# henrycharlesworth/settlers_of_catan_RL

Measured on AMD Instinct MI355X. Metric: Catan env-steps/sec at 65k parallel games, higher is better.
Workload: dtype u8/u32 (integer bitboards); 1 GPU; configs[1]: 65 536 parallel envs per GPU, random policy, step+mask only, bit-exact vs CPU oracle; games_per_gpu=65536, games_total=65536, validate_actions=True, auto_reset=True, parallelism=games sharded over 1 GPU(s), no collective

## Files before the change

settlers_of_catan_rl_amd/csrc/catan_kernels.hip:

```cpp
#include <hip/hip_runtime.h>
#include <stdint.h>

#include "catan_state.h"

#define CATAN_TABLE static __device__ __constant__ const
#define CATAN_FN static __device__ __forceinline__
#define CATAN_TOPOLOGY_CODE
#include "catan_topology.inc"

namespace catan {

#define DEVI __device__ __forceinline__

constexpr int BLOCK = 256;
constexpr u64 ALL54 = (1ull << 54) - 1;

constexpr int MT_RING = 8192, MT_AHEAD = 6144, MT_AHEAD_PY = 1024;
struct MtGen { u32 mt[624]; u32 idx; u32 produced; u32 ring[MT_RING]; };
struct MtPair { MtGen np, py; u32 cons_py; };
struct BoardCfg {
    int32_t randomise;
    int32_t fixed_terrain;
    int32_t fixed_numbers;
    int8_t terrain[19];
    int8_t numbers[18];
    int8_t pad_[7];
};
constexpr int MAX_BOARD_CFGS = 16;
struct Ctx {
    u32* R;
    long N;
    long n;
    u32 key0, key1;
    u64 env_id0;
    MtPair* mt;
    const BoardCfg* bcfg;
    const u8* bcfg_idx;
};

template <class D>
struct StOps {
// ... 1053 lines not shown
    const long i = (long)blockIdx.x * BLOCK + threadIdx.x;
    if (i >= rows * MASK_BITS) return;
    const long r = i / MASK_BITS;
    const int j = (int)(i - r * MASK_BITS);
    const long e = games != nullptr ? (long)games[r] : r;
    float v;
    if (e < 0 || e >= n || (busy != nullptr && busy[e] != 0)) v = j == M0 + T_ENDTURN ? 1.0f : 0.0f;
    else v = (float)((mpk[e * MPK_STRIDE + (j >> 5)] >> (j & 31)) & 1u);
    out[i] = v;
}

__global__ __launch_bounds__(BLOCK) void k_copy_masks11(const u32* __restrict__ mpk, long n, u32* __restrict__ out) {
    const long i = (long)blockIdx.x * BLOCK + threadIdx.x;
    if (i >= n * 11) return;
    const long e = i / 11;
    out[i] = mpk[e * MPK_STRIDE + (int)(i - e * 11)];
}
__global__ __launch_bounds__(256) void k_masked_row_store(unsigned char* __restrict__ dst, const unsigned char* __restrict__ src,
                                                          const long long* __restrict__ t, const unsigned char* __restrict__ sel,
                                                          long row_bytes, long step_stride_bytes) {
    const long r = blockIdx.x;
    if (!sel[r]) return;
    unsigned char* d = dst + t[r] * step_stride_bytes + r * row_bytes;
    const unsigned char* s = src + r * row_bytes;
    if ((((unsigned long long)d | (unsigned long long)s | (unsigned long long)row_bytes) & 3) == 0) {
        for (long i = threadIdx.x; i < row_bytes / 4; i += 256) reinterpret_cast<u32*>(d)[i] = reinterpret_cast<const u32*>(s)[i];
    } else if ((((unsigned long long)d | (unsigned long long)s | (unsigned long long)row_bytes) & 1) == 0) {
        for (long i = threadIdx.x; i < row_bytes / 2; i += 256) reinterpret_cast<unsigned short*>(d)[i] = reinterpret_cast<const unsigned short*>(s)[i];
    } else {
        for (long i = threadIdx.x; i < row_bytes; i += 256) d[i] = s[i];
    }
}

DEVI int nth_set(u64 v, int nth) {
    if (nth >= __popcll(v)) return -1;
    int pos = 0;
    u32 w = (u32)v;
    int c = __popc(w);
    if (nth >= c) { nth -= c; w = (u32)(v >> 32); pos = 32; }
    c = __popc(w & 0xFFFFu); if (nth >= c) { nth -= c; w >>= 16; pos += 16; }
    c = __popc(w & 0xFFu);   if (nth >= c) { nth -= c; w >>= 8;  pos += 8; }
    c = __popc(w & 0xFu);    if (nth >= c) { nth -= c; w >>= 4;  pos += 4; }
    c = __popc(w & 0x3u);    if (nth >= c) { nth -= c; w >>= 2;  pos += 2; }
    if (nth >= (int)(w & 1u)) pos += 1;
    return pos;
}
DEVI int pick64(u64 v, u32 w) {
    int k = __popcll(v);
    if (k == 0) return 0;
    return nth_set(v, (int)__umulhi(w, (u32)k));
}
template <class S>
DEVI int sample_random(const Ctx& c, const S& s, const u32 (&m)[MASK_WORDS], u32 step_idx, int (&a)[ACTION_WORDS],
                       u32* __restrict__ pctr, u8* __restrict__ busy, int tag_now, int tag_now2) {
#pragma unroll
    for (int i = 0; i < ACTION_WORDS; i++) a[i] = 0;
    if (pctr != nullptr) {
        const u32 own = pctr[s.e];
        int b = busy[s.e];
        if (b >= 2 && (b == tag_now || b == tag_now2)) { busy[s.e] = 0; b = 0; }
        if (b) { a[0] = -1; return -1; }
        step_idx = own;
        pctr[s.e] = step_idx + 1;
    }
    u64 id = c.env_id0 + (u64)s.e;
    u32 w[8];
    {
        u32 o[4];
        philox4x32_10(2 * step_idx, 1u, (u32)id, (u32)(id >> 32), c.key0, c.key1, o);
        w[0] = o[0]; w[1] = o[1]; w[2] = o[2]; w[3] = o[3];
    }
    int t = pick64(getr<M0, 13>(m), w[0]);
    a[0] = t;
    switch (t) {
    case T_SETTLE: a[1] = pick64(getr<M1, 54>(m), w[1]); break;
    case T_CITY: a[1] = pick64(getr<M1 + 54, 54>(m), w[1]); break;
    case T_ROAD: {
        u64 lo = getr<M2, 64>(m), hi = getr<M2 + 64, 9>(m);
        int k = __popcll(lo) + __popcll(hi);
        int nth = k ? (int)__umulhi(w[1], (u32)k) : 0;
        int nlo = __popcll(lo);
        a[2] = k == 0 ? 0 : (nth < nlo ? nth_set(lo, nth) : 64 + nth_set(hi, nth - nlo));
        break;
    }
    case T_ROBBER: a[3] = pick64(getr<M3, 19>(m), w[1]); break;
    case T_PLAYDEV:
        a[4] = pick64(getr<M4, 5>(m), w[1]);
        if (a[4] == C_MONO) a[15] = pick64(getr<M9 + 10, 5>(m), w[2]);
        else if (a[4] == C_YOP) { a[15] = pick64(getr<M9 + 15, 5>(m), w[2]); a[16] = pick64(getr<M10, 5>(m), w[3]); }
        break;
    case T_EXCHANGE: a[15] = pick64(getr<M9, 5>(m), w[1]); a[16] = pick64(getr<M10, 5>(m), w[2]); break;
    case T_PROPOSE: {
        {
            u32 o[4];
            philox4x32_10(2 * step_idx + 1, 1u, (u32)id, (u32)(id >> 32), c.key0, c.key1, o);
            w[4] = o[0]; w[5] = o[1]; w[6] = o[2]; w[7] = o[3];
        }
        int pid = s.b(B_GO);
        int hand[5], tot = 0;
#pragma unroll
        for (int r = 0; r < 5; r++) { hand[r] = s.res(pid, r); tot += hand[r]; }
        a[6] = (int)__umulhi(w[1], 3u);
        int n_give = 1 + (int)(w[2] & 1u), n_recv = 1 + (int)((w[2] >> 1) & 1u);
        if (n_give > tot) n_give = tot;
#pragma unroll
        for (int i = 0; i < 2; i++) if (i < n_give) {
            int nth = (int)__umulhi(w[3 + i], (u32)tot), r = 0;
            bool found = false;
#pragma unroll
            for (int k = 0; k < 5; k++) if (!found) { if (nth < hand[k]) { r = k; found = true; } else nth -= hand[k]; }
            a[7 + i] = r + 1;
#pragma unroll
            for (int k = 0; k < 5; k++) hand[k] -= (k == r) ? 1 : 0;
            tot--;
        }
#pragma unroll
        for (int i = 0; i < 2; i++) if (i < n_recv) a[11 + i] = 1 + (int)__umulhi(w[5 + i], 5u);
        break;
    }
    case T_RESPOND: a[5] = pick64(getr<M5, 2>(m), w[1]); break;
    case T_STEAL: a[6] = pick64(getr<M6 + 3, 3>(m), w[1]); break;
    case T_DISCARD: a[17] = pick64(getr<M11, 5>(m), w[1]); break;
    default: break;
    }
    return t;
}
template <class S>
DEVI bool action_valid(const S& s, const int (&a)[ACTION_WORDS]) {
    const int t = a[0];
    if (t < 0 || t > 12) return false;
    int cnt[5] = { 0, 0, 0, 0, 0 };
    if (t == T_STEAL && (a[6] < 0 || a[6] > 2)) return false;
    if (t == T_PLAYDEV) {
        if (a[4] == C_MONO && (a[15] < 0 || a[15] > 4)) return false;
        if (a[4] == C_YOP && (a[15] < 0 || a[15] > 4 || a[16] < 0 || a[16] > 4)) return false;
    }
    if (t == T_EXCHANGE && (a[15] < 0 || a[15] > 4 || a[16] < 0 || a[16] > 4)) return false;
    if (t == T_PROPOSE) {
        if (a[6] < 0 || a[6] > 2) return false;
        bool stop = false;
#pragma unroll
        for (int i = 0; i < 4; i++) {
            const int v = a[7 + i];
            if (v == 0) stop = true;
            if (!stop) {
                if (v < 0 || v > 5) return false;
#pragma unroll
                for (int k = 0; k < 5; k++) cnt[k] += (k == v - 1) ? 1 : 0;
            }
        }
        stop = false;
#pragma unroll
        for (int i = 0; i < 4; i++) { const int v = a[11 + i]; if (v == 0) stop = true; if (!stop && (v < 0 || v > 5)) return false; }
    }
    if (t == T_RESPOND && (a[5] < 0 || a[5] > 1)) return false;
    if (t == T_DISCARD && (a[17] < 0 || a[17] > 4)) return false;
// ... 1756 lines not shown
```

settlers_of_catan_rl_amd/csrc/catan_topology.inc:

```
CATAN_TABLE uint8_t TILE_CORNER[19][6] = {
  {0, 1, 2, 3, 4, 5},
  {6, 5, 4, 7, 8, 9},
  {10, 9, 8, 11, 12, 13},
  {2, 14, 15, 16, 17, 3},
  {4, 3, 17, 18, 19, 7},
  {8, 7, 19, 20, 21, 11},
  {12, 11, 21, 22, 23, 24},
  {15, 25, 26, 27, 28, 16},
  {17, 16, 28, 29, 30, 18},
  {19, 18, 30, 31, 32, 20},
  {21, 20, 32, 33, 34, 22},
  {23, 22, 34, 35, 36, 37},
  {28, 27, 38, 39, 40, 29},
  {30, 29, 40, 41, 42, 31},
  {32, 31, 42, 43, 44, 33},
  {34, 33, 44, 45, 46, 35},
  {40, 39, 47, 48, 49, 41},
  {42, 41, 49, 50, 51, 43},
  {44, 43, 51, 52, 53, 45},
};
CATAN_TABLE uint8_t EDGE_CORNER[72][2] = {
  {2, 3},
  {3, 4},
  {1, 2},
// ... 214 lines not shown
  {9, 13, 14},
  {9, 10, 14},
  {10, 14, 15},
  {10, 11, 15},
  {11, 15, 255},
  {11, 255, 255},
  {11, 255, 255},
  {12, 255, 255},
  {12, 16, 255},
  {12, 13, 16},
  {13, 16, 17},
  {13, 14, 17},
  {14, 17, 18},
  {14, 15, 18},
  {15, 18, 255},
  {15, 255, 255},
  {16, 255, 255},
  {16, 255, 255},
  {16, 17, 255},
  {17, 255, 255},
  {17, 18, 255},
  {18, 255, 255},
  {18, 255, 255},
};
CATAN_TABLE uint8_t CORNER_HSLOT[54] = {0, 0, 255, 255, 255, 255, 1, 255, 255, 1, 255, 255, 2, 255, 8, 8, 255, 255, 255, 255, 255, 255, 255, 255, 2, 255, 255, 7, 255, 255, 255, 255, 255, 255, 255, 255, 3, 3, 7, 255, 255, 255, 255, 255, 255, 4, 4, 6, 6, 255, 5, 5, 255, 255};
CATAN_TABLE uint8_t PLACEMENT[19] = {0, 3, 7, 12, 16, 17, 18, 15, 11, 6, 2, 1, 4, 8, 13, 14, 10, 5, 9};
CATAN_TABLE uint32_t TILE_NBR_MASK[19] = {0x1au, 0x35u, 0x62u, 0x191u, 0x32bu, 0x656u, 0xc24u, 0x1108u, 0x3298u, 0x6530u, 0xca60u, 0x8440u, 0x12180u, 0x35300u, 0x6a600u, 0x44c00u, 0x23000u, 0x56000u, 0x2c000u};
CATAN_TABLE uint64_t TILE_CORNER_MASK[19] = {0x3full, 0x3f0ull, 0x3f00ull, 0x3c00cull, 0xe0098ull, 0x380980ull, 0x1e01800ull, 0x1e018000ull, 0x70070000ull, 0x1c01c0000ull, 0x700700000ull, 0x3c00c00000ull, 0x1c038000000ull, 0x700e0000000ull, 0x1c0380000000ull, 0x700e00000000ull, 0x3838000000000ull, 0xe0e0000000000ull, 0x38380000000000ull};
CATAN_TABLE uint64_t CORNER_NBR_MASK[54] = {0x22ull, 0x5ull, 0x400aull, 0x20014ull, 0xa8ull, 0x51ull, 0x220ull, 0x80110ull, 0xa80ull, 0x540ull, 0x2200ull, 0x201100ull, 0x1002800ull, 0x1400ull, 0x8004ull, 0x2014000ull, 0x10028000ull, 0x50008ull, 0x400a0000ull, 0x140080ull, 0x100280000ull, 0x500800ull, 0x400a00000ull, 0x2001400000ull, 0x801000ull, 0x4008000ull, 0xa000000ull, 0x4014000000ull, 0x28010000ull, 0x10050000000ull, 0xa0040000ull, 0x40140000000ull, 0x280100000ull, 0x100500000000ull, 0xa00400000ull, 0x401400000000ull, 0x2800000000ull, 0x1000800000ull, 0x8008000000ull, 0x814000000000ull, 0x28020000000ull, 0x2050000000000ull, 0xa0080000000ull, 0x8140000000000ull, 0x280200000000ull, 0x20500000000000ull, 0x200800000000ull, 0x1008000000000ull, 0x2800000000000ull, 0x5020000000000ull, 0xa000000000000ull, 0x14080000000000ull, 0x28000000000000ull, 0x10200000000000ull};
CATAN_TABLE uint64_t EDGE_CORNER_MASK[72] = {0xcull, 0x18ull, 0x6ull, 0x30ull, 0x3ull, 0x21ull, 0x90ull, 0x180ull, 0x300ull, 0x60ull, 0x240ull, 0x900ull, 0x1800ull, 0x3000ull, 0x600ull, 0x2400ull, 0x18000ull, 0x30000ull, 0xc000ull, 0x20008ull, 0x4004ull, 0x60000ull, 0xc0000ull, 0x80080ull, 0x180000ull, 0x300000ull, 0x200800ull, 0x600000ull, 0xc00000ull, 0x1800000ull, 0x1001000ull, 0xc000000ull, 0x18000000ull, 0x6000000ull, 0x10010000ull, 0x2008000ull, 0x30000000ull, 0x60000000ull, 0x40040000ull, 0xc0000000ull, 0x180000000ull, 0x100100000ull, 0x300000000ull, 0x600000000ull, 0x400400000ull, 0xc00000000ull, 0x1800000000ull, 0x3000000000ull, 0x2000800000ull, 0xc000000000ull, 0x18000000000ull, 0x4008000000ull, 0x10020000000ull, 0x30000000000ull, 0x60000000000ull, 0x40080000000ull, 0xc0000000000ull, 0x180000000000ull, 0x100200000000ull, 0x300000000000ull, 0x600000000000ull, 0x400800000000ull, 0x1800000000000ull, 0x3000000000000ull, 0x808000000000ull, 0x2020000000000ull, 0x6000000000000ull, 0xc000000000000ull, 0x8080000000000ull, 0x18000000000000ull, 0x30000000000000ull, 0x20200000000000ull};
#ifdef CATAN_TOPOLOGY_CODE
CATAN_FN uint64_t topo_blocked(uint64_t occ) {
    const uint32_t ol = (uint32_t)occ, oh = (uint32_t)(occ >> 32);
    uint32_t bl = ol, bh = oh, m;
    m = 0u - ((ol >> 0) & 1u); bl |= m & 0x22u;
    m = 0u - ((ol >> 1) & 1u); bl |= m & 0x5u;
    m = 0u - ((ol >> 2) & 1u); bl |= m & 0x400au;
    m = 0u - ((ol >> 3) & 1u); bl |= m & 0x20014u;
    m = 0u - ((ol >> 4) & 1u); bl |= m & 0xa8u;
    m = 0u - ((ol >> 5) & 1u); bl |= m & 0x51u;
    m = 0u - ((ol >> 6) & 1u); bl |= m & 0x220u;
    m = 0u - ((ol >> 7) & 1u); bl |= m & 0x80110u;
    m = 0u - ((ol >> 8) & 1u); bl |= m & 0xa80u;
    m = 0u - ((ol >> 9) & 1u); bl |= m & 0x540u;
    m = 0u - ((ol >> 10) & 1u); bl |= m & 0x2200u;
    m = 0u - ((ol >> 11) & 1u); bl |= m & 0x201100u;
    m = 0u - ((ol >> 12) & 1u); bl |= m & 0x1002800u;
    m = 0u - ((ol >> 13) & 1u); bl |= m & 0x1400u;
    m = 0u - ((ol >> 14) & 1u); bl |= m & 0x8004u;
    m = 0u - ((ol >> 15) & 1u); bl |= m & 0x2014000u;
    m = 0u - ((ol >> 16) & 1u); bl |= m & 0x10028000u;
    m = 0u - ((ol >> 17) & 1u); bl |= m & 0x50008u;
    m = 0u - ((ol >> 18) & 1u); bl |= m & 0x400a0000u;
    m = 0u - ((ol >> 19) & 1u); bl |= m & 0x140080u;
    m = 0u - ((ol >> 20) & 1u); bl |= m & 0x280000u; bh |= m & 0x1u;
    m = 0u - ((ol >> 21) & 1u); bl |= m & 0x500800u;
    m = 0u - ((ol >> 22) & 1u); bl |= m & 0xa00000u; bh |= m & 0x4u;
    m = 0u - ((ol >> 23) & 1u); bl |= m & 0x1400000u; bh |= m & 0x20u;
    m = 0u - ((ol >> 24) & 1u); bl |= m & 0x801000u;
    m = 0u - ((ol >> 25) & 1u); bl |= m & 0x4008000u;
    m = 0u - ((ol >> 26) & 1u); bl |= m & 0xa000000u;
    m = 0u - ((ol >> 27) & 1u); bl |= m & 0x14000000u; bh |= m & 0x40u;
    m = 0u - ((ol >> 28) & 1u); bl |= m & 0x28010000u;
    m = 0u - ((ol >> 29) & 1u); bl |= m & 0x50000000u; bh |= m & 0x100u;
    m = 0u - ((ol >> 30) & 1u); bl |= m & 0xa0040000u;
    m = 0u - ((ol >> 31) & 1u); bl |= m & 0x40000000u; bh |= m & 0x401u;
    m = 0u - ((oh >> 0) & 1u); bl |= m & 0x80100000u; bh |= m & 0x2u;
    m = 0u - ((oh >> 1) & 1u); bh |= m & 0x1005u;
    m = 0u - ((oh >> 2) & 1u); bl |= m & 0x400000u; bh |= m & 0xau;
    m = 0u - ((oh >> 3) & 1u); bh |= m & 0x4014u;
    m = 0u - ((oh >> 4) & 1u); bh |= m & 0x28u;
    m = 0u - ((oh >> 5) & 1u); bl |= m & 0x800000u; bh |= m & 0x10u;
    m = 0u - ((oh >> 6) & 1u); bl |= m & 0x8000000u; bh |= m & 0x80u;
    m = 0u - ((oh >> 7) & 1u); bh |= m & 0x8140u;
    m = 0u - ((oh >> 8) & 1u); bl |= m & 0x20000000u; bh |= m & 0x280u;
    m = 0u - ((oh >> 9) & 1u); bh |= m & 0x20500u;
    m = 0u - ((oh >> 10) & 1u); bl |= m & 0x80000000u; bh |= m & 0xa00u;
    m = 0u - ((oh >> 11) & 1u); bh |= m & 0x81400u;
    m = 0u - ((oh >> 12) & 1u); bh |= m & 0x2802u;
    m = 0u - ((oh >> 13) & 1u); bh |= m & 0x205000u;
    m = 0u - ((oh >> 14) & 1u); bh |= m & 0x2008u;
    m = 0u - ((oh >> 15) & 1u); bh |= m & 0x10080u;
    m = 0u - ((oh >> 16) & 1u); bh |= m & 0x28000u;
    m = 0u - ((oh >> 17) & 1u); bh |= m & 0x50200u;
    m = 0u - ((oh >> 18) & 1u); bh |= m & 0xa0000u;
    m = 0u - ((oh >> 19) & 1u); bh |= m & 0x140800u;
    m = 0u - ((oh >> 20) & 1u); bh |= m & 0x280000u;
    m = 0u - ((oh >> 21) & 1u); bh |= m & 0x102000u;
    return (uint64_t)bl | ((uint64_t)bh << 32);
}
CATAN_FN uint64_t topo_touched(uint64_t lo, uint32_t hi) {
    const uint32_t e0 = (uint32_t)lo, e1 = (uint32_t)(lo >> 32), e2 = hi;
    uint32_t tl = 0, th = 0, m;
    m = 0u - ((e0 >> 0) & 1u); tl |= m & 0xcu;
    m = 0u - ((e0 >> 1) & 1u); tl |= m & 0x18u;
    m = 0u - ((e0 >> 2) & 1u); tl |= m & 0x6u;
    m = 0u - ((e0 >> 3) & 1u); tl |= m & 0x30u;
    m = 0u - ((e0 >> 4) & 1u); tl |= m & 0x3u;
    m = 0u - ((e0 >> 5) & 1u); tl |= m & 0x21u;
    m = 0u - ((e0 >> 6) & 1u); tl |= m & 0x90u;
    m = 0u - ((e0 >> 7) & 1u); tl |= m & 0x180u;
    m = 0u - ((e0 >> 8) & 1u); tl |= m & 0x300u;
    m = 0u - ((e0 >> 9) & 1u); tl |= m & 0x60u;
    m = 0u - ((e0 >> 10) & 1u); tl |= m & 0x240u;
    m = 0u - ((e0 >> 11) & 1u); tl |= m & 0x900u;
    m = 0u - ((e0 >> 12) & 1u); tl |= m & 0x1800u;
    m = 0u - ((e0 >> 13) & 1u); tl |= m & 0x3000u;
    m = 0u - ((e0 >> 14) & 1u); tl |= m & 0x600u;
    m = 0u - ((e0 >> 15) & 1u); tl |= m & 0x2400u;
    m = 0u - ((e0 >> 16) & 1u); tl |= m & 0x18000u;
    m = 0u - ((e0 >> 17) & 1u); tl |= m & 0x30000u;
    m = 0u - ((e0 >> 18) & 1u); tl |= m & 0xc000u;
    m = 0u - ((e0 >> 19) & 1u); tl |= m & 0x20008u;
    m = 0u - ((e0 >> 20) & 1u); tl |= m & 0x4004u;
    m = 0u - ((e0 >> 21) & 1u); tl |= m & 0x60000u;
    m = 0u - ((e0 >> 22) & 1u); tl |= m & 0xc0000u;
    m = 0u - ((e0 >> 23) & 1u); tl |= m & 0x80080u;
    m = 0u - ((e0 >> 24) & 1u); tl |= m & 0x180000u;
    m = 0u - ((e0 >> 25) & 1u); tl |= m & 0x300000u;
    m = 0u - ((e0 >> 26) & 1u); tl |= m & 0x200800u;
    m = 0u - ((e0 >> 27) & 1u); tl |= m & 0x600000u;
    m = 0u - ((e0 >> 28) & 1u); tl |= m & 0xc00000u;
    m = 0u - ((e0 >> 29) & 1u); tl |= m & 0x1800000u;
    m = 0u - ((e0 >> 30) & 1u); tl |= m & 0x1001000u;
    m = 0u - ((e0 >> 31) & 1u); tl |= m & 0xc000000u;
    m = 0u - ((e1 >> 0) & 1u); tl |= m & 0x18000000u;
    m = 0u - ((e1 >> 1) & 1u); tl |= m & 0x6000000u;
    m = 0u - ((e1 >> 2) & 1u); tl |= m & 0x10010000u;
    m = 0u - ((e1 >> 3) & 1u); tl |= m & 0x2008000u;
    m = 0u - ((e1 >> 4) & 1u); tl |= m & 0x30000000u;
    m = 0u - ((e1 >> 5) & 1u); tl |= m & 0x60000000u;
    m = 0u - ((e1 >> 6) & 1u); tl |= m & 0x40040000u;
    m = 0u - ((e1 >> 7) & 1u); tl |= m & 0xc0000000u;
    m = 0u - ((e1 >> 8) & 1u); tl |= m & 0x80000000u; th |= m & 0x1u;
    m = 0u - ((e1 >> 9) & 1u); tl |= m & 0x100000u; th |= m & 0x1u;
    m = 0u - ((e1 >> 10) & 1u); th |= m & 0x3u;
    m = 0u - ((e1 >> 11) & 1u); th |= m & 0x6u;
    m = 0u - ((e1 >> 12) & 1u); tl |= m & 0x400000u; th |= m & 0x4u;
    m = 0u - ((e1 >> 13) & 1u); th |= m & 0xcu;
    m = 0u - ((e1 >> 14) & 1u); th |= m & 0x18u;
    m = 0u - ((e1 >> 15) & 1u); th |= m & 0x30u;
    m = 0u - ((e1 >> 16) & 1u); tl |= m & 0x800000u; th |= m & 0x20u;
    m = 0u - ((e1 >> 17) & 1u); th |= m & 0xc0u;
    m = 0u - ((e1 >> 18) & 1u); th |= m & 0x180u;
    m = 0u - ((e1 >> 19) & 1u); tl |= m & 0x8000000u; th |= m & 0x40u;
    m = 0u - ((e1 >> 20) & 1u); tl |= m & 0x20000000u; th |= m & 0x100u;
    m = 0u - ((e1 >> 21) & 1u); th |= m & 0x300u;
    m = 0u - ((e1 >> 22) & 1u); th |= m & 0x600u;
    m = 0u - ((e1 >> 23) & 1u); tl |= m & 0x80000000u; th |= m & 0x400u;
    m = 0u - ((e1 >> 24) & 1u); th |= m & 0xc00u;
    m = 0u - ((e1 >> 25) & 1u); th |= m & 0x1800u;
    m = 0u - ((e1 >> 26) & 1u); th |= m & 0x1002u;
    m = 0u - ((e1 >> 27) & 1u); th |= m & 0x3000u;
    m = 0u - ((e1 >> 28) & 1u); th |= m & 0x6000u;
    m = 0u - ((e1 >> 29) & 1u); th |= m & 0x4008u;
    m = 0u - ((e1 >> 30) & 1u); th |= m & 0x18000u;
    m = 0u - ((e1 >> 31) & 1u); th |= m & 0x30000u;
    m = 0u - ((e2 >> 0) & 1u); th |= m & 0x8080u;
    m = 0u - ((e2 >> 1) & 1u); th |= m & 0x20200u;
    m = 0u - ((e2 >> 2) & 1u); th |= m & 0x60000u;
    m = 0u - ((e2 >> 3) & 1u); th |= m & 0xc0000u;
    m = 0u - ((e2 >> 4) & 1u); th |= m & 0x80800u;
    m = 0u - ((e2 >> 5) & 1u); th |= m & 0x180000u;
    m = 0u - ((e2 >> 6) & 1u); th |= m & 0x300000u;
    m = 0u - ((e2 >> 7) & 1u); th |= m & 0x202000u;
    return (uint64_t)tl | ((uint64_t)th << 32);
}
CATAN_FN void topo_edges_at(uint64_t anchors, uint64_t& lo, uint32_t& hi) {
    const uint32_t al = (uint32_t)anchors, ah = (uint32_t)(anchors >> 32);
    uint32_t e0 = 0, e1 = 0, e2 = 0, m;
    m = 0u - ((al >> 0) & 1u); e0 |= m & 0x30u;
    m = 0u - ((al >> 1) & 1u); e0 |= m & 0x14u;
    m = 0u - ((al >> 2) & 1u); e0 |= m & 0x100005u;
    m = 0u - ((al >> 3) & 1u); e0 |= m & 0x80003u;
    m = 0u - ((al >> 4) & 1u); e0 |= m & 0x4au;
    m = 0u - ((al >> 5) & 1u); e0 |= m & 0x228u;
    m = 0u - ((al >> 6) & 1u); e0 |= m & 0x600u;
    m = 0u - ((al >> 7) & 1u); e0 |= m & 0x8000c0u;
    m = 0u - ((al >> 8) & 1u); e0 |= m & 0x980u;
    m = 0u - ((al >> 9) & 1u); e0 |= m & 0x4500u;
    m = 0u - ((al >> 10) & 1u); e0 |= m & 0xc000u;
    m = 0u - ((al >> 11) & 1u); e0 |= m & 0x4001800u;
    m = 0u - ((al >> 12) & 1u); e0 |= m & 0x40003000u;
    m = 0u - ((al >> 13) & 1u); e0 |= m & 0xa000u;
    m = 0u - ((al >> 14) & 1u); e0 |= m & 0x140000u;
    m = 0u - ((al >> 15) & 1u); e0 |= m & 0x50000u; e1 |= m & 0x8u;
    m = 0u - ((al >> 16) & 1u); e0 |= m & 0x30000u; e1 |= m & 0x4u;
    m = 0u - ((al >> 17) & 1u); e0 |= m & 0x2a0000u;
    m = 0u - ((al >> 18) & 1u); e0 |= m & 0x600000u; e1 |= m & 0x40u;
    m = 0u - ((al >> 19) & 1u); e0 |= m & 0x1c00000u;
    m = 0u - ((al >> 20) & 1u); e0 |= m & 0x3000000u; e1 |= m & 0x200u;
    m = 0u - ((al >> 21) & 1u); e0 |= m & 0xe000000u;
    m = 0u - ((al >> 22) & 1u); e0 |= m & 0x18000000u; e1 |= m & 0x1000u;
    m = 0u - ((al >> 23) & 1u); e0 |= m & 0x30000000u; e1 |= m & 0x10000u;
    m = 0u - ((al >> 24) & 1u); e0 |= m & 0x60000000u;
    m = 0u - ((al >> 25) & 1u); e1 |= m & 0xau;
    m = 0u - ((al >> 26) & 1u); e0 |= m & 0x80000000u; e1 |= m & 0x2u;
    m = 0u - ((al >> 27) & 1u); e0 |= m & 0x80000000u; e1 |= m & 0x80001u;
    m = 0u - ((al >> 28) & 1u); e1 |= m & 0x15u;
    m = 0u - ((al >> 29) & 1u); e1 |= m & 0x100030u;
    m = 0u - ((al >> 30) & 1u); e1 |= m & 0xe0u;
    m = 0u - ((al >> 31) & 1u); e1 |= m & 0x800180u;
    m = 0u - ((ah >> 0) & 1u); e1 |= m & 0x700u;
    m = 0u - ((ah >> 1) & 1u); e1 |= m & 0x4000c00u;
    m = 0u - ((ah >> 2) & 1u); e1 |= m & 0x3800u;
    m = 0u - ((ah >> 3) & 1u); e1 |= m & 0x20006000u;
    m = 0u - ((ah >> 4) & 1u); e1 |= m & 0xc000u;
    m = 0u - ((ah >> 5) & 1u); e1 |= m & 0x18000u;
    m = 0u - ((ah >> 6) & 1u); e1 |= m & 0xa0000u;
    m = 0u - ((ah >> 7) & 1u); e1 |= m & 0x60000u; e2 |= m & 0x1u;
    m = 0u - ((ah >> 8) & 1u); e1 |= m & 0x340000u;
    m = 0u - ((ah >> 9) & 1u); e1 |= m & 0x600000u; e2 |= m & 0x2u;
    m = 0u - ((ah >> 10) & 1u); e1 |= m & 0x1c00000u;
    m = 0u - ((ah >> 11) & 1u); e1 |= m & 0x3000000u; e2 |= m & 0x10u;
    m = 0u - ((ah >> 12) & 1u); e1 |= m & 0xe000000u;
    m = 0u - ((ah >> 13) & 1u); e1 |= m & 0x18000000u; e2 |= m & 0x80u;
    m = 0u - ((ah >> 14) & 1u); e1 |= m & 0x30000000u;
    m = 0u - ((ah >> 15) & 1u); e1 |= m & 0x40000000u; e2 |= m & 0x1u;
    m = 0u - ((ah >> 16) & 1u); e1 |= m & 0xc0000000u;
    m = 0u - ((ah >> 17) & 1u); e1 |= m & 0x80000000u; e2 |= m & 0x6u;
    m = 0u - ((ah >> 18) & 1u); e2 |= m & 0xcu;
    m = 0u - ((ah >> 19) & 1u); e2 |= m & 0x38u;
    m = 0u - ((ah >> 20) & 1u); e2 |= m & 0x60u;
    m = 0u - ((ah >> 21) & 1u); e2 |= m & 0xc0u;
    lo = (uint64_t)e0 | ((uint64_t)e1 << 32); hi = e2;
}
CATAN_FN uint32_t topo_tiles_at(uint64_t occ) {
    const uint32_t ol = (uint32_t)occ, oh = (uint32_t)(occ >> 32);
    uint32_t t = 0;
    t |= ((ol & 0x3fu)) ? 0x1u : 0u;
    t |= ((ol & 0x3f0u)) ? 0x2u : 0u;
    t |= ((ol & 0x3f00u)) ? 0x4u : 0u;
    t |= ((ol & 0x3c00cu)) ? 0x8u : 0u;
    t |= ((ol & 0xe0098u)) ? 0x10u : 0u;
    t |= ((ol & 0x380980u)) ? 0x20u : 0u;
    t |= ((ol & 0x1e01800u)) ? 0x40u : 0u;
    t |= ((ol & 0x1e018000u)) ? 0x80u : 0u;
    t |= ((ol & 0x70070000u)) ? 0x100u : 0u;
    t |= ((ol & 0xc01c0000u) | (oh & 0x1u)) ? 0x200u : 0u;
    t |= ((ol & 0x700000u) | (oh & 0x7u)) ? 0x400u : 0u;
    t |= ((ol & 0xc00000u) | (oh & 0x3cu)) ? 0x800u : 0u;
    t |= ((ol & 0x38000000u) | (oh & 0x1c0u)) ? 0x1000u : 0u;
    t |= ((ol & 0xe0000000u) | (oh & 0x700u)) ? 0x2000u : 0u;
    t |= ((ol & 0x80000000u) | (oh & 0x1c03u)) ? 0x4000u : 0u;
    t |= ((oh & 0x700eu)) ? 0x8000u : 0u;
    t |= ((oh & 0x38380u)) ? 0x10000u : 0u;
    t |= ((oh & 0xe0e00u)) ? 0x20000u : 0u;
    t |= ((oh & 0x383800u)) ? 0x40000u : 0u;
    return t;
}
CATAN_FN uint64_t topo_tile_corners(int t) {
    uint64_t m = 0;
    if (t == 0) m = 0x3full;
    if (t == 1) m = 0x3f0ull;
    if (t == 2) m = 0x3f00ull;
    if (t == 3) m = 0x3c00cull;
    if (t == 4) m = 0xe0098ull;
// ... 64 lines not shown
```

Measured before the change: 1.055 billion env-steps/s.

## Replace per-bit topology masks with shift-grouped ORs and branchless action sampling

The topology adjacency functions (blocked corners, touched corners, edges at anchors) are rewritten. The old form did one mask-and-OR per source bit; the new form groups the bits that share the same shift distance into a single shift-and-mask. This cuts roughly 50–70 dependent ops per call down to about 20–40. Separately, the random action sampler drops its switch over action types in favour of a table-driven, branchless extraction of the relevant mask window (up to 73 bits) followed by a single pick, which reduces wavefront divergence across games. The risk is subtle bit-mapping errors in the regenerated masks, which would break bit-exactness against the CPU oracle.

```diff
diff --git a/settlers_of_catan_rl_amd/csrc/catan_kernels.hip b/settlers_of_catan_rl_amd/csrc/catan_kernels.hip
--- a/settlers_of_catan_rl_amd/csrc/catan_kernels.hip
+++ b/settlers_of_catan_rl_amd/csrc/catan_kernels.hip
@@ -7,6 +7,8 @@
 #define CATAN_FN static __device__ __forceinline__
 #define CATAN_TOPOLOGY_CODE
 #include "catan_topology.inc"
+#define CATAN_PICK_FN static __device__ __forceinline__
+#include "catan_pick.h"
 
 namespace catan {
 
@@ -1126,24 +1128,24 @@
     }
 }
 
-DEVI int nth_set(u64 v, int nth) {
-    if (nth >= __popcll(v)) return -1;
-    int pos = 0;
-    u32 w = (u32)v;
-    int c = __popc(w);
-    if (nth >= c) { nth -= c; w = (u32)(v >> 32); pos = 32; }
-    c = __popc(w & 0xFFFFu); if (nth >= c) { nth -= c; w >>= 16; pos += 16; }
-    c = __popc(w & 0xFFu);   if (nth >= c) { nth -= c; w >>= 8;  pos += 8; }
-    c = __popc(w & 0xFu);    if (nth >= c) { nth -= c; w >>= 4;  pos += 4; }
-    c = __popc(w & 0x3u);    if (nth >= c) { nth -= c; w >>= 2;  pos += 2; }
-    if (nth >= (int)(w & 1u)) pos += 1;
-    return pos;
-}
-DEVI int pick64(u64 v, u32 w) {
-    int k = __popcll(v);
-    if (k == 0) return 0;
-    return nth_set(v, (int)__umulhi(w, (u32)k));
-}
+using catan_pick::pick32;
+using catan_pick::pick73;
+struct FirstPick { short off, width, slot; };
+constexpr FirstPick FIRST_PICK[13] = {
+    { M1, 54, 1 },
+    { M2, 73, 2 },
+    { M1 + 54, 54, 1 },
+    { 0, 0, 0 },
+    { M4, 5, 4 },
+    { M9, 5, 15 },
+    { 0, 0, 0 },
+    { M5, 2, 5 },
+    { M3, 19, 3 },
+    { 0, 0, 0 },
+    { 0, 0, 0 },
+    { M6 + 3, 3, 6 },
+    { M11, 5, 17 },
+};
 template <class S>
 DEVI int sample_random(const Ctx& c, const S& s, const u32 (&m)[MASK_WORDS], u32 step_idx, int (&a)[ACTION_WORDS],
                        u32* __restrict__ pctr, u8* __restrict__ busy, int tag_now, int tag_now2) {
@@ -1164,27 +1166,39 @@
         philox4x32_10(2 * step_idx, 1u, (u32)id, (u32)(id >> 32), c.key0, c.key1, o);
         w[0] = o[0]; w[1] = o[1]; w[2] = o[2]; w[3] = o[3];
     }
-    int t = pick64(getr<M0, 13>(m), w[0]);
+    const int t = pick32((u32)getr<M0, 13>(m), w[0]);
     a[0] = t;
-    switch (t) {
-    case T_SETTLE: a[1] = pick64(getr<M1, 54>(m), w[1]); break;
-    case T_CITY: a[1] = pick64(getr<M1 + 54, 54>(m), w[1]); break;
-    case T_ROAD: {
-        u64 lo = getr<M2, 64>(m), hi = getr<M2 + 64, 9>(m);
-        int k = __popcll(lo) + __popcll(hi);
-        int nth = k ? (int)__umulhi(w[1], (u32)k) : 0;
-        int nlo = __popcll(lo);
-        a[2] = k == 0 ? 0 : (nth < nlo ? nth_set(lo, nth) : 64 + nth_set(hi, nth - nlo));
-        break;
-    }
-    case T_ROBBER: a[3] = pick64(getr<M3, 19>(m), w[1]); break;
-    case T_PLAYDEV:
-        a[4] = pick64(getr<M4, 5>(m), w[1]);
-        if (a[4] == C_MONO) a[15] = pick64(getr<M9 + 10, 5>(m), w[2]);
-        else if (a[4] == C_YOP) { a[15] = pick64(getr<M9 + 15, 5>(m), w[2]); a[16] = pick64(getr<M10, 5>(m), w[3]); }
-        break;
-    case T_EXCHANGE: a[15] = pick64(getr<M9, 5>(m), w[1]); a[16] = pick64(getr<M10, 5>(m), w[2]); break;
-    case T_PROPOSE: {
+    {
+        u32 x0 = 0, x1 = 0, x2 = 0;
+        int r = 0, width = 0;
+#pragma unroll
+        for (int i = 0; i < 13; i++) {
+            const int off = FIRST_PICK[i].off, wd = FIRST_PICK[i].width;
+            if (wd > 0 && t == i) {
+                x0 = m[off >> 5];
+                if ((off & 31) + wd > 32) x1 = m[(off >> 5) + 1];
+                if ((off & 31) + wd > 64) x2 = m[(off >> 5) + 2];
+                r = off & 31; width = wd;
+            }
+        }
+        u64 lo;
+        u32 hi;
+        catan_pick::extract73(x0, x1, x2, r, width, lo, hi);
+        const int p = pick73(lo, hi, w[1]);
+#pragma unroll
+        for (int i = 0; i < 13; i++) if (FIRST_PICK[i].width > 0 && t == i) a[FIRST_PICK[i].slot] = p;
+    }
+    {
+        const int card = a[4];
+        u32 v2 = 0, v3 = 0;
+        if (t == T_PLAYDEV && card == C_MONO) v2 = (u32)getr<M9 + 10, 5>(m);
+        if (t == T_PLAYDEV && card == C_YOP) { v2 = (u32)getr<M9 + 15, 5>(m); v3 = (u32)getr<M10, 5>(m); }
+        if (t == T_EXCHANGE) v2 = (u32)getr<M10, 5>(m);
+        const int p2 = pick32(v2, w[2]), p3 = pick32(v3, w[3]);
+        if (t == T_PLAYDEV) { a[15] = p2; a[16] = p3; }
+        if (t == T_EXCHANGE) a[16] = p2;
+    }
+    if (t == T_PROPOSE) {
         {
             u32 o[4];
             philox4x32_10(2 * step_idx + 1, 1u, (u32)id, (u32)(id >> 32), c.key0, c.key1, o);
@@ -1210,12 +1224,6 @@
         }
 #pragma unroll
         for (int i = 0; i < 2; i++) if (i < n_recv) a[11 + i] = 1 + (int)__umulhi(w[5 + i], 5u);
-        break;
-    }
-    case T_RESPOND: a[5] = pick64(getr<M5, 2>(m), w[1]); break;
-    case T_STEAL: a[6] = pick64(getr<M6 + 3, 3>(m), w[1]); break;
-    case T_DISCARD: a[17] = pick64(getr<M11, 5>(m), w[1]); break;
-    default: break;
     }
     return t;
 }
diff --git a/settlers_of_catan_rl_amd/csrc/catan_pick.h b/settlers_of_catan_rl_amd/csrc/catan_pick.h
--- /dev/null
+++ b/settlers_of_catan_rl_amd/csrc/catan_pick.h
@@ -0,0 +1,50 @@
+#pragma once
+#include <stdint.h>
+
+#ifndef CATAN_PICK_FN
+#define CATAN_PICK_FN static inline
+#endif
+
+namespace catan_pick {
+
+CATAN_PICK_FN uint32_t mulhi(uint32_t a, uint32_t b) { return (uint32_t)(((uint64_t)a * b) >> 32); }
+
+CATAN_PICK_FN int rank32(uint32_t w, int nth) {
+    int pos = 0, c;
+    c = __builtin_popcount(w & 0xFFFFu); if (nth >= c) { nth -= c; w >>= 16; pos += 16; }
+    c = __builtin_popcount(w & 0xFFu);   if (nth >= c) { nth -= c; w >>= 8;  pos += 8; }
+    c = __builtin_popcount(w & 0xFu);    if (nth >= c) { nth -= c; w >>= 4;  pos += 4; }
+    c = __builtin_popcount(w & 0x3u);    if (nth >= c) { nth -= c; w >>= 2;  pos += 2; }
+    if (nth >= (int)(w & 1u)) pos += 1;
+    return pos;
+}
+CATAN_PICK_FN int rank64(uint64_t v, int nth) {
+    const int c = __builtin_popcount((uint32_t)v);
+    const bool up = nth >= c;
+    return (up ? 32 : 0) + rank32(up ? (uint32_t)(v >> 32) : (uint32_t)v, up ? nth - c : nth);
+}
+CATAN_PICK_FN int nth_set(uint64_t v, int nth) { return nth >= __builtin_popcountll(v) ? -1 : rank64(v, nth); }
+CATAN_PICK_FN int pick64(uint64_t v, uint32_t w) {
+    const int k = __builtin_popcountll(v);
+    if (k == 0) return 0;
+    return rank64(v, (int)mulhi(w, (uint32_t)k));
+}
+CATAN_PICK_FN int pick32(uint32_t v, uint32_t w) {
+    const int k = __builtin_popcount(v);
+    if (k == 0) return 0;
+    return rank32(v, (int)mulhi(w, (uint32_t)k));
+}
+CATAN_PICK_FN int pick73(uint64_t lo, uint32_t hi, uint32_t w) {
+    const int nlo = __builtin_popcountll(lo), k = nlo + __builtin_popcount(hi);
+    const int nth = (int)mulhi(w, (uint32_t)k);
+    const bool up = nth >= nlo;
+    const int p = rank64(up ? (uint64_t)hi : lo, up ? nth - nlo : nth);
+    return k == 0 ? 0 : (up ? 64 : 0) + p;
+}
+CATAN_PICK_FN void extract73(uint32_t x0, uint32_t x1, uint32_t x2, int r, int width, uint64_t& lo, uint32_t& hi) {
+    const uint32_t a = (uint32_t)((((uint64_t)x1 << 32) | x0) >> r), b = (uint32_t)((((uint64_t)x2 << 32) | x1) >> r);
+    lo = ((uint64_t)a | ((uint64_t)b << 32)) & (width >= 64 ? ~0ull : ((1ull << (width & 63)) - 1));
+    hi = (x2 >> r) & (width > 64 ? (1u << ((width - 64) & 31)) - 1 : 0u);
+}
+
+}
diff --git a/settlers_of_catan_rl_amd/csrc/catan_topology.inc b/settlers_of_catan_rl_amd/csrc/catan_topology.inc
--- a/settlers_of_catan_rl_amd/csrc/catan_topology.inc
+++ b/settlers_of_catan_rl_amd/csrc/catan_topology.inc
@@ -270,197 +270,114 @@
 #ifdef CATAN_TOPOLOGY_CODE
 CATAN_FN uint64_t topo_blocked(uint64_t occ) {
     const uint32_t ol = (uint32_t)occ, oh = (uint32_t)(occ >> 32);
-    uint32_t bl = ol, bh = oh, m;
-    m = 0u - ((ol >> 0) & 1u); bl |= m & 0x22u;
-    m = 0u - ((ol >> 1) & 1u); bl |= m & 0x5u;
-    m = 0u - ((ol >> 2) & 1u); bl |= m & 0x400au;
-    m = 0u - ((ol >> 3) & 1u); bl |= m & 0x20014u;
-    m = 0u - ((ol >> 4) & 1u); bl |= m & 0xa8u;
-    m = 0u - ((ol >> 5) & 1u); bl |= m & 0x51u;
-    m = 0u - ((ol >> 6) & 1u); bl |= m & 0x220u;
-    m = 0u - ((ol >> 7) & 1u); bl |= m & 0x80110u;
-    m = 0u - ((ol >> 8) & 1u); bl |= m & 0xa80u;
-    m = 0u - ((ol >> 9) & 1u); bl |= m & 0x540u;
-    m = 0u - ((ol >> 10) & 1u); bl |= m & 0x2200u;
-    m = 0u - ((ol >> 11) & 1u); bl |= m & 0x201100u;
-    m = 0u - ((ol >> 12) & 1u); bl |= m & 0x1002800u;
-    m = 0u - ((ol >> 13) & 1u); bl |= m & 0x1400u;
-    m = 0u - ((ol >> 14) & 1u); bl |= m & 0x8004u;
-    m = 0u - ((ol >> 15) & 1u); bl |= m & 0x2014000u;
-    m = 0u - ((ol >> 16) & 1u); bl |= m & 0x10028000u;
-    m = 0u - ((ol >> 17) & 1u); bl |= m & 0x50008u;
-    m = 0u - ((ol >> 18) & 1u); bl |= m & 0x400a0000u;
-    m = 0u - ((ol >> 19) & 1u); bl |= m & 0x140080u;
-    m = 0u - ((ol >> 20) & 1u); bl |= m & 0x280000u; bh |= m & 0x1u;
-    m = 0u - ((ol >> 21) & 1u); bl |= m & 0x500800u;
-    m = 0u - ((ol >> 22) & 1u); bl |= m & 0xa00000u; bh |= m & 0x4u;
-    m = 0u - ((ol >> 23) & 1u); bl |= m & 0x1400000u; bh |= m & 0x20u;
-    m = 0u - ((ol >> 24) & 1u); bl |= m & 0x801000u;
-    m = 0u - ((ol >> 25) & 1u); bl |= m & 0x4008000u;
-    m = 0u - ((ol >> 26) & 1u); bl |= m & 0xa000000u;
-    m = 0u - ((ol >> 27) & 1u); bl |= m & 0x14000000u; bh |= m & 0x40u;
-    m = 0u - ((ol >> 28) & 1u); bl |= m & 0x28010000u;
-    m = 0u - ((ol >> 29) & 1u); bl |= m & 0x50000000u; bh |= m & 0x100u;
-    m = 0u - ((ol >> 30) & 1u); bl |= m & 0xa0040000u;
-    m = 0u - ((ol >> 31) & 1u); bl |= m & 0x40000000u; bh |= m & 0x401u;
-    m = 0u - ((oh >> 0) & 1u); bl |= m & 0x80100000u; bh |= m & 0x2u;
-    m = 0u - ((oh >> 1) & 1u); bh |= m & 0x1005u;
-    m = 0u - ((oh >> 2) & 1u); bl |= m & 0x400000u; bh |= m & 0xau;
-    m = 0u - ((oh >> 3) & 1u); bh |= m & 0x4014u;
-    m = 0u - ((oh >> 4) & 1u); bh |= m & 0x28u;
-    m = 0u - ((oh >> 5) & 1u); bl |= m & 0x800000u; bh |= m & 0x10u;
-    m = 0u - ((oh >> 6) & 1u); bl |= m & 0x8000000u; bh |= m & 0x80u;
-    m = 0u - ((oh >> 7) & 1u); bh |= m & 0x8140u;
-    m = 0u - ((oh >> 8) & 1u); bl |= m & 0x20000000u; bh |= m & 0x280u;
-    m = 0u - ((oh >> 9) & 1u); bh |= m & 0x20500u;
-    m = 0u - ((oh >> 10) & 1u); bl |= m & 0x80000000u; bh |= m & 0xa00u;
-    m = 0u - ((oh >> 11) & 1u); bh |= m & 0x81400u;
-    m = 0u - ((oh >> 12) & 1u); bh |= m & 0x2802u;
-    m = 0u - ((oh >> 13) & 1u); bh |= m & 0x205000u;
-    m = 0u - ((oh >> 14) & 1u); bh |= m & 0x2008u;
-    m = 0u - ((oh >> 15) & 1u); bh |= m & 0x10080u;
-    m = 0u - ((oh >> 16) & 1u); bh |= m & 0x28000u;
-    m = 0u - ((oh >> 17) & 1u); bh |= m & 0x50200u;
-    m = 0u - ((oh >> 18) & 1u); bh |= m & 0xa0000u;
-    m = 0u - ((oh >> 19) & 1u); bh |= m & 0x140800u;
-    m = 0u - ((oh >> 20) & 1u); bh |= m & 0x280000u;
-    m = 0u - ((oh >> 21) & 1u); bh |= m & 0x102000u;
+    uint32_t bl = ol, bh = oh;
+    bl |= (uint32_t)((((uint64_t)oh << 32) | ol) >> 14) & 0x800008u;
+    bl |= (uint32_t)((((uint64_t)oh << 32) | ol) >> 12) & 0x551084u;
+    bl |= (oh << 21) & 0xa8000000u;
+    bh |= (oh >> 11) & 0xau;
+    bl |= (ol >> 10) & 0x8800u;
+    bh |= (oh >> 8) & 0x2a80u;
+    bl |= (ol >> 5) & 0x1u;
+    bl |= (ol >> 3) & 0x550u;
+    bl |= (uint32_t)((((uint64_t)oh << 32) | ol) >> 1) & 0xfeffdbbfu;
+    bh |= (oh >> 1) & 0x1fbfdfu;
+    bl |= (ol << 1) & 0xfdffb77eu;
+    bh |= (uint32_t)((((uint64_t)oh << 32) | ol) >> 31) & 0x3f7fbfu;
+    bl |= (ol << 3) & 0x2a80u;
+    bl |= (ol << 5) & 0x20u;
+    bh |= (oh << 8) & 0x2a8000u;
+    bl |= (ol << 10) & 0x2200000u;
+    bh |= (uint32_t)((((uint64_t)oh << 32) | ol) >> 21) & 0x5540u;
+    bl |= (ol << 12) & 0x51084000u;
+    bh |= (ol >> 20) & 0x5u;
+    bl |= (ol << 14) & 0x20000u;
+    bh |= (ol >> 18) & 0x20u;
     return (uint64_t)bl | ((uint64_t)bh << 32);
 }
 CATAN_FN uint64_t topo_touched(uint64_t lo, uint32_t hi) {
     const uint32_t e0 = (uint32_t)lo, e1 = (uint32_t)(lo >> 32), e2 = hi;
-    uint32_t tl = 0, th = 0, m;
-    m = 0u - ((e0 >> 0) & 1u); tl |= m & 0xcu;
-    m = 0u - ((e0 >> 1) & 1u); tl |= m & 0x18u;
-    m = 0u - ((e0 >> 2) & 1u); tl |= m & 0x6u;
-    m = 0u - ((e0 >> 3) & 1u); tl |= m & 0x30u;
-    m = 0u - ((e0 >> 4) & 1u); tl |= m & 0x3u;
-    m = 0u - ((e0 >> 5) & 1u); tl |= m & 0x21u;
-    m = 0u - ((e0 >> 6) & 1u); tl |= m & 0x90u;
-    m = 0u - ((e0 >> 7) & 1u); tl |= m & 0x180u;
-    m = 0u - ((e0 >> 8) & 1u); tl |= m & 0x300u;
-    m = 0u - ((e0 >> 9) & 1u); tl |= m & 0x60u;
-    m = 0u - ((e0 >> 10) & 1u); tl |= m & 0x240u;
-    m = 0u - ((e0 >> 11) & 1u); tl |= m & 0x900u;
-    m = 0u - ((e0 >> 12) & 1u); tl |= m & 0x1800u;
-    m = 0u - ((e0 >> 13) & 1u); tl |= m & 0x3000u;
-    m = 0u - ((e0 >> 14) & 1u); tl |= m & 0x600u;
-    m = 0u - ((e0 >> 15) & 1u); tl |= m & 0x2400u;
-    m = 0u - ((e0 >> 16) & 1u); tl |= m & 0x18000u;
-    m = 0u - ((e0 >> 17) & 1u); tl |= m & 0x30000u;
-    m = 0u - ((e0 >> 18) & 1u); tl |= m & 0xc000u;
-    m = 0u - ((e0 >> 19) & 1u); tl |= m & 0x20008u;
-    m = 0u - ((e0 >> 20) & 1u); tl |= m & 0x4004u;
-    m = 0u - ((e0 >> 21) & 1u); tl |= m & 0x60000u;
-    m = 0u - ((e0 >> 22) & 1u); tl |= m & 0xc0000u;
-    m = 0u - ((e0 >> 23) & 1u); tl |= m & 0x80080u;
-    m = 0u - ((e0 >> 24) & 1u); tl |= m & 0x180000u;
-    m = 0u - ((e0 >> 25) & 1u); tl |= m & 0x300000u;
-    m = 0u - ((e0 >> 26) & 1u); tl |= m & 0x200800u;
-    m = 0u - ((e0 >> 27) & 1u); tl |= m & 0x600000u;
-    m = 0u - ((e0 >> 28) & 1u); tl |= m & 0xc00000u;
-    m = 0u - ((e0 >> 29) & 1u); tl |= m & 0x1800000u;
-    m = 0u - ((e0 >> 30) & 1u); tl |= m & 0x1001000u;
-    m = 0u - ((e0 >> 31) & 1u); tl |= m & 0xc000000u;
-    m = 0u - ((e1 >> 0) & 1u); tl |= m & 0x18000000u;
-    m = 0u - ((e1 >> 1) & 1u); tl |= m & 0x6000000u;
-    m = 0u - ((e1 >> 2) & 1u); tl |= m & 0x10010000u;
-    m = 0u - ((e1 >> 3) & 1u); tl |= m & 0x2008000u;
-    m = 0u - ((e1 >> 4) & 1u); tl |= m & 0x30000000u;
-    m = 0u - ((e1 >> 5) & 1u); tl |= m & 0x60000000u;
-    m = 0u - ((e1 >> 6) & 1u); tl |= m & 0x40040000u;
-    m = 0u - ((e1 >> 7) & 1u); tl |= m & 0xc0000000u;
-    m = 0u - ((e1 >> 8) & 1u); tl |= m & 0x80000000u; th |= m & 0x1u;
-    m = 0u - ((e1 >> 9) & 1u); tl |= m & 0x100000u; th |= m & 0x1u;
-    m = 0u - ((e1 >> 10) & 1u); th |= m & 0x3u;
-    m = 0u - ((e1 >> 11) & 1u); th |= m & 0x6u;
-    m = 0u - ((e1 >> 12) & 1u); tl |= m & 0x400000u; th |= m & 0x4u;
-    m = 0u - ((e1 >> 13) & 1u); th |= m & 0xcu;
-    m = 0u - ((e1 >> 14) & 1u); th |= m & 0x18u;
-    m = 0u - ((e1 >> 15) & 1u); th |= m & 0x30u;
-    m = 0u - ((e1 >> 16) & 1u); tl |= m & 0x800000u; th |= m & 0x20u;
-    m = 0u - ((e1 >> 17) & 1u); th |= m & 0xc0u;
-    m = 0u - ((e1 >> 18) & 1u); th |= m & 0x180u;
-    m = 0u - ((e1 >> 19) & 1u); tl |= m & 0x8000000u; th |= m & 0x40u;
-    m = 0u - ((e1 >> 20) & 1u); tl |= m & 0x20000000u; th |= m & 0x100u;
-    m = 0u - ((e1 >> 21) & 1u); th |= m & 0x300u;
-    m = 0u - ((e1 >> 22) & 1u); th |= m & 0x600u;
-    m = 0u - ((e1 >> 23) & 1u); tl |= m & 0x80000000u; th |= m & 0x400u;
-    m = 0u - ((e1 >> 24) & 1u); th |= m & 0xc00u;
-    m = 0u - ((e1 >> 25) & 1u); th |= m & 0x1800u;
-    m = 0u - ((e1 >> 26) & 1u); th |= m & 0x1002u;
-    m = 0u - ((e1 >> 27) & 1u); th |= m & 0x3000u;
-    m = 0u - ((e1 >> 28) & 1u); th |= m & 0x6000u;
-    m = 0u - ((e1 >> 29) & 1u); th |= m & 0x4008u;
-    m = 0u - ((e1 >> 30) & 1u); th |= m & 0x18000u;
-    m = 0u - ((e1 >> 31) & 1u); th |= m & 0x30000u;
-    m = 0u - ((e2 >> 0) & 1u); th |= m & 0x8080u;
-    m = 0u - ((e2 >> 1) & 1u); th |= m & 0x20200u;
-    m = 0u - ((e2 >> 2) & 1u); th |= m & 0x60000u;
-    m = 0u - ((e2 >> 3) & 1u); th |= m & 0xc0000u;
-    m = 0u - ((e2 >> 4) & 1u); th |= m & 0x80800u;
-    m = 0u - ((e2 >> 5) & 1u); th |= m & 0x180000u;
-    m = 0u - ((e2 >> 6) & 1u); th |= m & 0x300000u;
-    m = 0u - ((e2 >> 7) & 1u); th |= m & 0x202000u;
+    uint32_t tl = 0, th = 0;
+    th |= (uint32_t)((((uint64_t)e2 << 32) | e1) >> 26) & 0x2008u;
+    tl |= (e1 << 7) & 0x800000u;
+    th |= (uint32_t)((((uint64_t)e2 << 32) | e1) >> 25) & 0x882u;
+    tl |= (e1 << 8) & 0x88000000u;
+    th |= (e2 << 8) & 0x200u;
+    tl |= (e1 << 9) & 0x20000000u;
+    tl |= (e1 << 10) & 0x400000u;
+    tl |= (e1 << 11) & 0x100000u;
+    tl |= (e1 << 12) & 0x48000u;
+    tl |= (uint32_t)((((uint64_t)e1 << 32) | e0) >> 18) & 0x11004u;
+    th |= (e2 << 14) & 0x380000u;
+    th |= (e2 << 15) & 0x3e8000u;
+    tl |= (e0 >> 16) & 0x88u;
+    th |= (e2 << 16) & 0xe0000u;
+    tl |= (e0 >> 15) & 0x800u;
+    th |= (e1 >> 15) & 0x1f000u;
+    th |= (e1 >> 14) & 0x37c00u;
+    th |= (e1 >> 13) & 0x1f40u;
+    th |= (e1 >> 12) & 0x700u;
+    th |= (e1 >> 11) & 0xfcu;
+    tl |= (e1 << 22) & 0x2000000u;
+    th |= (e1 >> 10) & 0x1bfu;
+    tl |= (e1 << 23) & 0xc0000000u;
+    th |= (e1 >> 9) & 0x7u;
+    tl |= (e1 << 24) & 0xf2000000u;
+    th |= (e1 >> 8) & 0x1u;
+    tl |= (e1 << 25) & 0x64000000u;
+    tl |= (uint32_t)((((uint64_t)e1 << 32) | e0) >> 6) & 0x11e04000u;
+    tl |= (uint32_t)((((uint64_t)e1 << 32) | e0) >> 5) & 0xdf80601u;
+    tl |= (uint32_t)((((uint64_t)e1 << 32) | e0) >> 4) & 0x183e4461u;
+    tl |= (e0 >> 3) & 0xc8142u;
+    tl |= (e0 >> 2) & 0x22010u;
+    tl |= (e0 >> 1) & 0x19a02u;
+    tl |= e0 & 0x339a4u;
+    tl |= (e0 << 1) & 0x390u;
+    tl |= (e0 << 2) & 0x2cu;
+    tl |= (e0 << 3) & 0x18u;
     return (uint64_t)tl | ((uint64_t)th << 32);
 }
 CATAN_FN void topo_edges_at(uint64_t anchors, uint64_t& lo, uint32_t& hi) {
     const uint32_t al = (uint32_t)anchors, ah = (uint32_t)(anchors >> 32);
-    uint32_t e0 = 0, e1 = 0, e2 = 0, m;
-    m = 0u - ((al >> 0) & 1u); e0 |= m & 0x30u;
-    m = 0u - ((al >> 1) & 1u); e0 |= m & 0x14u;
-    m = 0u - ((al >> 2) & 1u); e0 |= m & 0x100005u;
-    m = 0u - ((al >> 3) & 1u); e0 |= m & 0x80003u;
-    m = 0u - ((al >> 4) & 1u); e0 |= m & 0x4au;
-    m = 0u - ((al >> 5) & 1u); e0 |= m & 0x228u;
-    m = 0u - ((al >> 6) & 1u); e0 |= m & 0x600u;
-    m = 0u - ((al >> 7) & 1u); e0 |= m & 0x8000c0u;
-    m = 0u - ((al >> 8) & 1u); e0 |= m & 0x980u;
-    m = 0u - ((al >> 9) & 1u); e0 |= m & 0x4500u;
-    m = 0u - ((al >> 10) & 1u); e0 |= m & 0xc000u;
-    m = 0u - ((al >> 11) & 1u); e0 |= m & 0x4001800u;
-    m = 0u - ((al >> 12) & 1u); e0 |= m & 0x40003000u;
-    m = 0u - ((al >> 13) & 1u); e0 |= m & 0xa000u;
-    m = 0u - ((al >> 14) & 1u); e0 |= m & 0x140000u;
-    m = 0u - ((al >> 15) & 1u); e0 |= m & 0x50000u; e1 |= m & 0x8u;
-    m = 0u - ((al >> 16) & 1u); e0 |= m & 0x30000u; e1 |= m & 0x4u;
-    m = 0u - ((al >> 17) & 1u); e0 |= m & 0x2a0000u;
-    m = 0u - ((al >> 18) & 1u); e0 |= m & 0x600000u; e1 |= m & 0x40u;
-    m = 0u - ((al >> 19) & 1u); e0 |= m & 0x1c00000u;
-    m = 0u - ((al >> 20) & 1u); e0 |= m & 0x3000000u; e1 |= m & 0x200u;
-    m = 0u - ((al >> 21) & 1u); e0 |= m & 0xe000000u;
-    m = 0u - ((al >> 22) & 1u); e0 |= m & 0x18000000u; e1 |= m & 0x1000u;
-    m = 0u - ((al >> 23) & 1u); e0 |= m & 0x30000000u; e1 |= m & 0x10000u;
-    m = 0u - ((al >> 24) & 1u); e0 |= m & 0x60000000u;
-    m = 0u - ((al >> 25) & 1u); e1 |= m & 0xau;
-    m = 0u - ((al >> 26) & 1u); e0 |= m & 0x80000000u; e1 |= m & 0x2u;
-    m = 0u - ((al >> 27) & 1u); e0 |= m & 0x80000000u; e1 |= m & 0x80001u;
-    m = 0u - ((al >> 28) & 1u); e1 |= m & 0x15u;
-    m = 0u - ((al >> 29) & 1u); e1 |= m & 0x100030u;
-    m = 0u - ((al >> 30) & 1u); e1 |= m & 0xe0u;
-    m = 0u - ((al >> 31) & 1u); e1 |= m & 0x800180u;
-    m = 0u - ((ah >> 0) & 1u); e1 |= m & 0x700u;
-    m = 0u - ((ah >> 1) & 1u); e1 |= m & 0x4000c00u;
-    m = 0u - ((ah >> 2) & 1u); e1 |= m & 0x3800u;
-    m = 0u - ((ah >> 3) & 1u); e1 |= m & 0x20006000u;
-    m = 0u - ((ah >> 4) & 1u); e1 |= m & 0xc000u;
-    m = 0u - ((ah >> 5) & 1u); e1 |= m & 0x18000u;
-    m = 0u - ((ah >> 6) & 1u); e1 |= m & 0xa0000u;
-    m = 0u - ((ah >> 7) & 1u); e1 |= m & 0x60000u; e2 |= m & 0x1u;
-    m = 0u - ((ah >> 8) & 1u); e1 |= m & 0x340000u;
-    m = 0u - ((ah >> 9) & 1u); e1 |= m & 0x600000u; e2 |= m & 0x2u;
-    m = 0u - ((ah >> 10) & 1u); e1 |= m & 0x1c00000u;
-    m = 0u - ((ah >> 11) & 1u); e1 |= m & 0x3000000u; e2 |= m & 0x10u;
-    m = 0u - ((ah >> 12) & 1u); e1 |= m & 0xe000000u;
-    m = 0u - ((ah >> 13) & 1u); e1 |= m & 0x18000000u; e2 |= m & 0x80u;
-    m = 0u - ((ah >> 14) & 1u); e1 |= m & 0x30000000u;
-    m = 0u - ((ah >> 15) & 1u); e1 |= m & 0x40000000u; e2 |= m & 0x1u;
-    m = 0u - ((ah >> 16) & 1u); e1 |= m & 0xc0000000u;
-    m = 0u - ((ah >> 17) & 1u); e1 |= m & 0x80000000u; e2 |= m & 0x6u;
-    m = 0u - ((ah >> 18) & 1u); e2 |= m & 0xcu;
-    m = 0u - ((ah >> 19) & 1u); e2 |= m & 0x38u;
-    m = 0u - ((ah >> 20) & 1u); e2 |= m & 0x60u;
-    m = 0u - ((ah >> 21) & 1u); e2 |= m & 0xc0u;
+    uint32_t e0 = 0, e1 = 0, e2 = 0;
+    e0 |= (al >> 3) & 0x3u;
+    e0 |= (al >> 2) & 0xbu;
+    e0 |= (al >> 1) & 0x1c8u;
+    e0 |= al & 0x339a4u;
+    e0 |= (al << 1) & 0x33404u;
+    e0 |= (al << 2) & 0x88040u;
+    e0 |= (al << 3) & 0x640a10u;
+    e0 |= (al << 4) & 0x83e44610u;
+    e1 |= (al >> 28) & 0x1u;
+    e0 |= (al << 5) & 0xbf00c020u;
+    e1 |= (al >> 27) & 0x1u;
+    e0 |= (al << 6) & 0x78100000u;
+    e1 |= (al >> 26) & 0x4u;
+    e1 |= (al >> 25) & 0x32u;
+    e1 |= (uint32_t)((((uint64_t)ah << 32) | al) >> 24) & 0x1f2u;
+    e1 |= (uint32_t)((((uint64_t)ah << 32) | al) >> 23) & 0xf80u;
+    e1 |= (uint32_t)((((uint64_t)ah << 32) | al) >> 22) & 0x6fc08u;
+    e1 |= (ah << 11) & 0x7e000u;
+    e1 |= (ah << 12) & 0x700000u;
+    e1 |= (ah << 13) & 0x3e80000u;
+    e1 |= (ah << 14) & 0xdf000000u;
+    e0 |= (al << 15) & 0x4000000u;
+    e1 |= (ah << 15) & 0xf8000000u;
+    e0 |= (al << 16) & 0x880000u;
+    e2 |= (ah >> 16) & 0xeu;
+    e2 |= (ah >> 15) & 0x7du;
+    e0 |= (al << 18) & 0x40100000u;
+    e1 |= (al >> 14) & 0x4u;
+    e2 |= (ah >> 14) & 0xe0u;
+    e1 |= (al >> 12) & 0x48u;
+    e1 |= (al >> 11) & 0x200u;
+    e1 |= (al >> 10) & 0x1000u;
+    e1 |= (al >> 9) & 0x100000u;
+    e1 |= (al >> 8) & 0x880000u;
+    e2 |= (ah >> 8) & 0x2u;
+    e1 |= (uint32_t)((((uint64_t)ah << 32) | al) >> 7) & 0x4010000u;
+    e2 |= (ah >> 7) & 0x11u;
+    e1 |= (ah << 26) & 0x20000000u;
+    e2 |= (ah >> 6) & 0x80u;
     lo = (uint64_t)e0 | ((uint64_t)e1 << 32); hi = e2;
 }
 CATAN_FN uint32_t topo_tiles_at(uint64_t occ) {
```

Measured after the change: 1.059 billion env-steps/s, median of 4. Within noise of the previous version (+0.4%).
